# kekeliu-whu/MSF_LOAM

Hardware: AMD Instinct MI355X
Metric: scan-to-map registrations/s (higher is better)
Workload: dtype f64 (f32 kNN distances)

## Files before the change

msf_loam_amd/csrc/msfl_api_slam.inc:

```

#include "msfl_slam.cuh"

namespace {

struct SlamScanBuf {
  DevBuf in_pts, in_ring;
  DevBuf full, fring, curv, label, idx;
  DevBuf cnt;
  DevBuf ex_off;
  DevBuf sharp, ls, ls_ring, flat, lf, lf_ring;
  DevBuf map_ls, map_lf;
  DevBuf full_scan, full_map;
  DevBuf imu;
  int imu_mode = 0;
  DevBuf dqp;
  DevBuf odo_off, odo_status;
  DevBuf poses;
  PinBuf upload;
  int n = 0;
  hipEvent_t ev_odo = nullptr;
  hipEvent_t ev_pose = nullptr, ev_cready = nullptr, ev_match = nullptr, ev_cdone = nullptr;
  DevBuf vox_c, vox_s, vsum_c, vsum_s;
  DevBuf vmeta;
  hipEvent_t ev_feat = nullptr, ev_vox = nullptr;
// ... 119 lines not shown
  r->status_imu = cnt[SC_IMU_BAD] ? MSFL_BAD_ARG : 0;
  cnt[SC_IMU_BAD] = 0;
  r->status_clouds = cnt[SC_CLOUD_BAD] ? MSFL_BAD_ARG : 0;
  cnt[SC_CLOUD_BAD] = 0;
  r->reserved_ = 0;
  r->status_insert = (r->grid_corner[3] | r->grid_corner[4] | r->grid_surf[3] | r->grid_surf[4]) ? MSFL_CAPACITY : 0;
  if (r->odometry.status == 0 && *odo_status != 0) r->odometry.status = *odo_status;
}

msfl_status scan2scan_dyn(msfl_handle* h, const SlamScanBuf& last, const SlamScanBuf& cur, const SlamCaps& caps, double* d_pose, const RegSinks& sinks) {
  hipStream_t st = h->stream;
  const int B = 1;
  const int* d_off = cur.odo_off.as<int>();
  int* d_status = cur.odo_status.as<int>();
  const int n_rec_cap = caps.sharp + caps.flat;
  HIPCHK(h, h->records.reserve(((size_t)4 * caps.flat + (size_t)6 * caps.sharp + 8) * sizeof(double)));
  const BatchView bv = batch_view(cur.sharp.as<float4>(), cur.flat.as<float4>(), d_off + 4, 2, B, n_rec_cap, 0, 0, caps.flat, 1);
  OdomView ov;
  ov.last_ls = last.ls.as<float4>(); ov.last_ls_ring = last.ls_ring.as<uint16_t>(); ov.last_ls_off = d_off;
  ov.last_lf = last.lf.as<float4>(); ov.last_lf_ring = last.lf_ring.as<uint16_t>(); ov.last_lf_off = d_off + 2;
  ov.dist_sq_threshold = h->prm.odom_distance_sq_threshold;
  ov.nearby_scan = h->prm.odom_nearby_scan;
  const SolverParams sp = solver_params(h->prm, h->prm.odom_min_correspondences);
  const bool gate_fits_grid = h->prm.odom_distance_sq_threshold <= 35.9;
  const bool use_grid = gate_fits_grid && !h->odom_force_brute;
  OdomIndex oix{nullptr, nullptr, nullptr, nullptr, std::max(1, div_up(caps.flat, kOdomBlock / kSlamOdomLanes))};
  OdomIndex oie{nullptr, nullptr, nullptr, nullptr, std::max(1, div_up(caps.sharp, kOdomBlock / kSlamOdomLanes))};
  if (use_grid) {
    ScopedTimer timer(h, T_ODOM);
    HIPCHK(h, h->od[OD_TAB].reserve((size_t)B * kOdomTabStride * sizeof(unsigned)));
    HIPCHK(h, h->od[OD_SORTED].reserve((size_t)caps.less_flat * sizeof(float4)));
// ... 18 lines not shown
    ScopedTimer timer(h, T_ODOM);
    hipLaunchKernelGGL(assoc_scan2scan_kernel, dim3(div_up(n_rec_cap, 256), B), dim3(256), 0, st, bv, ov, (const double*)d_pose,
                       (const int*)d_status, h->records.as<double>(), oix.mode, oie.mode);
    if (use_grid) {
      const int plane_blocks = div_up(B, 8) * 8 * oix.tiles, edge_blocks = div_up(B, 8) * 8 * oie.tiles;
      hipLaunchKernelGGL((assoc_scan2scan_grid_kernel<kSlamOdomLanes>), dim3(plane_blocks + edge_blocks), dim3(kOdomBlock), 0, st, bv, ov, oix, oie,
                         plane_blocks, (const double*)d_pose, (const int*)d_status, h->records.as<double>());
    }
    return MSFL_OK;
  });
}

msfl_status scan2map_dyn(msfl_handle* h, const float4* d_corner, const float4* d_surf, const int* d_in_off, int cap_corner, int cap_surf,
                         double* d_pose, int* d_status, const RegSinks& sinks, const DeskewView* deskew = nullptr) {
  const int n_rec_cap = cap_corner + cap_surf;
  HIPCHK(h, h->records.reserve(((size_t)4 * cap_surf + (size_t)6 * cap_corner + 8) * sizeof(double)));
  HIPCHK(h, h->nn.reserve(std::max<size_t>(1, (size_t)n_rec_cap) * 5 * sizeof(int)));
  const BatchView bv = batch_view(d_corner, d_surf, d_in_off, 2, 1, n_rec_cap, 0, 0, cap_surf, 1);
  DeskewView dv{};
  if (deskew) {
    dv = *deskew;
    HIPCHK(h, h->pprime.reserve(std::max<size_t>(1, (size_t)n_rec_cap) * 3 * sizeof(double)));
    dv.pprime = h->pprime.as<double>();
  }
  return solve_outer<kSlamLmBlock>(h, 1, bv, dv.pprime, d_pose, d_status, sinks, solver_params(h->prm, 0), h->prm.outer_iterations, [&](int) {
    s_launch_assoc(h, bv, d_pose, d_status, deskew != nullptr, dv, n_rec_cap);
    return MSFL_OK;
  });
}

constexpr size_t kVoxScratchBytes = (size_t)65536 * 8 + (size_t)2 * 65536 * 2;
// ... 634 lines not shown
```

msf_loam_amd/csrc/msfl_kernels.cuh:

```cuda
#pragma once
#include <hip/hip_runtime.h>
#include <stdint.h>

#include "msfl_math.cuh"

namespace msfl {

#ifndef MSFL_GRID_XSUB
#define MSFL_GRID_XSUB 3
#endif
constexpr int kGridXSub = MSFL_GRID_XSUB;

struct GridDesc {
  float ox, oy, oz;
  float inv_cell;
  float inv_cell_x;
  int dx, dy, dz;
  int n_pts;
  int n_cells;
  int reach;
  int want_cells;
  float cell2, cellx2;
};

// ... 539 lines not shown
  return b;
}
__device__ __forceinline__ int find_scan(const int* __restrict__ rec_off, int n_scans, int g) {
  int lo = 0, hi = n_scans;
  while (hi - lo > 1) {
    const int mid = (lo + hi) >> 1;
    if (rec_off[mid] <= g) lo = mid; else hi = mid;
  }
  return lo;
}

__device__ __forceinline__ size_t feature_slot(const BatchView& bv, bool edge, int f) {
  return edge ? (size_t)(f - bv.c0) : (size_t)(bv.n_records - bv.n_surf_total) + (size_t)(f - bv.s0);
}

__device__ __forceinline__ size_t plane_rec_off(const BatchView& bv, int fi_surf) { return 4 * (size_t)(fi_surf - bv.s0); }
__device__ __forceinline__ size_t edge_rec_off(const BatchView& bv, int fi_corner) {
  return 4 * (size_t)bv.n_surf_total + 6 * (size_t)(fi_corner - bv.c0);
}

struct DeskewView {
  const double* corner_dq; const double* corner_dp;
  const double* surf_dq;   const double* surf_dp;
  const double* V;
  double G[3];
  const double* G_dev;
  double* pprime;
};

#ifndef MSFL_ASSOC_BLOCK
#define MSFL_ASSOC_BLOCK 64
#endif
constexpr int kAssocBlock = MSFL_ASSOC_BLOCK;
// ... 256 lines not shown
    if (DESKEW && fo.ok) {
      static_assert(!DESKEW || KIND == 0, "the de-skew branch runs the per-record kernel");
      const int fd = is_edge ? bv.corner_off[b] + local : bv.surf_off[b] + (local - nc);
      const double dt = (double)(is_edge ? bv.corner[fd].w : bv.surf[fd].w);
      const double* Vb = dv.V + 3 * (size_t)b;
      const double Gv[3] = {dv.G_dev ? dv.G_dev[0] : dv.G[0], dv.G_dev ? dv.G_dev[1] : dv.G[1], dv.G_dev ? dv.G_dev[2] : dv.G[2]};
      fo.C = fo.C - mk3(Vb[0] * dt - 0.5 * Gv[0] * dt * dt, Vb[1] * dt - 0.5 * Gv[1] * dt * dt,
                        Vb[2] * dt - 0.5 * Gv[2] * dt * dt);
    }
  }
  if (is_edge) {
    double* out = rec + edge_rec_off(bv, KIND == 0 ? bv.corner_off[b] + local : fi);
    out[0] = fo.C.x; out[1] = fo.C.y; out[2] = fo.C.z;
    out[3] = fo.N.x; out[4] = fo.N.y; out[5] = fo.N.z;
  } else {
    double* out = rec + plane_rec_off(bv, KIND == 0 ? bv.surf_off[b] + (local - nc) : fi);
    out[0] = fo.N.x; out[1] = fo.N.y; out[2] = fo.N.z; out[3] = dot(fo.N, fo.C);
  }
  if (KIND == 0 && full) {
    double* o = full + 6 * (size_t)g;
    o[0] = fo.C.x; o[1] = fo.C.y; o[2] = fo.C.z; o[3] = fo.N.x; o[4] = fo.N.y; o[5] = fo.N.z;
  }
}

template <bool DESKEW>
__global__ void __launch_bounds__(kAssocBlock, MSFL_FIT_WAVES)
fit_scan2map_kernel(BatchView bv, const float4* __restrict__ map_c, const float4* __restrict__ map_s,
                    const int* __restrict__ nn, double line_ratio, double plane_tol, DeskewView dv,
                    double* __restrict__ rec, double* __restrict__ full) {
  fit_one<DESKEW, 0>(bv, map_c, map_s, nn, line_ratio, plane_tol, dv, rec, full, (int)blockIdx.x);
}
#ifndef MSFL_FIT_SPLIT_WAVES
// ... 7 lines not shown
  else fit_one<false, 2>(bv, map_c, map_s, nn, line_ratio, plane_tol, dv, rec, full, (int)blockIdx.x - edge_blocks);
}

__global__ void __launch_bounds__(256) pack_records_kernel(BatchView bv, const double* __restrict__ full, double* __restrict__ rec) {
  const int g = blockIdx.x * blockDim.x + threadIdx.x;
  if (g >= batch_records(bv)) return;
  const int b = find_scan_wave(bv.rec_off, bv.n_scans, g);
  const int local = g - bv.rec_off[b];
  const int nc = bv.corner_off[b + 1] - bv.corner_off[b];
  const double* in = full + 6 * (size_t)g;
  if (local < nc) {
    double* out = rec + edge_rec_off(bv, bv.corner_off[b] + local);
#pragma unroll
    for (int k = 0; k < 6; k++) out[k] = in[k];
  } else {
    double* out = rec + plane_rec_off(bv, bv.surf_off[b] + (local - nc));
    out[0] = in[3]; out[1] = in[4]; out[2] = in[5]; out[3] = in[3] * in[0] + in[4] * in[1] + in[5] * in[2];
  }
}


struct SolverParams {
  int    max_iterations;
  double huber;
  double radius0, radius_max, radius_min;
  double min_relative_decrease, min_diag, max_diag;
  double ftol, gtol, ptol;
  int    max_invalid;
  int    min_correspondences;
};

struct DevMatchInfo {
// ... 32 lines not shown
#ifndef MSFL_LM_BLOCK
#define MSFL_LM_BLOCK 128
#endif
constexpr int kLmBlock = MSFL_LM_BLOCK;
#ifndef MSFL_ODOM_LM_BLOCK
#define MSFL_ODOM_LM_BLOCK 128
#endif
constexpr int kOdomLmBlock = MSFL_ODOM_LM_BLOCK;
#ifndef MSFL_LM_GROUP_SMALL
#define MSFL_LM_GROUP_SMALL 8
#endif
#ifndef MSFL_LM_GROUP_LARGE
#define MSFL_LM_GROUP_LARGE 4
#endif
constexpr int lm_load_group(int block) { return block >= 512 ? MSFL_LM_GROUP_LARGE : MSFL_LM_GROUP_SMALL; }
constexpr int lm_plane_cache(int block) {
#ifdef MSFL_LM_PLANE_CACHE
  return block == 256 ? MSFL_LM_PLANE_CACHE : block == 128 ? 832 : block == 512 ? 3072 : 384;
#else
  return block == 256 ? 1728 : block == 128 ? 832 : block == 512 ? 3072 : 384;
#endif
}
template <int BLOCK>
struct PlaneCache {
  static constexpr int kPlanes = lm_plane_cache(BLOCK);
  double nx[kPlanes], ny[kPlanes], nz[kPlanes], d0[kPlanes];
  float px[kPlanes], py[kPlanes], pz[kPlanes];
};

constexpr int kEdgeListMax = 1024;
struct EdgeList {
  unsigned mask[kEdgeListMax / 32];
  unsigned short idx[kEdgeListMax];
  int n;
};

#ifdef MSFL_LM_PROFILE
__device__ unsigned long long g_lm_prof[8];
#define LM_T(x) const unsigned long long x = wall_clock64()
#ifndef MSFL_LM_PROFILE_BLOCK
#define MSFL_LM_PROFILE_BLOCK 0
#endif
#define LM_ADD(k, v) if (threadIdx.x == 0 && (MSFL_LM_PROFILE_BLOCK == 0 || MSFL_LM_PROFILE_BLOCK == (int)blockDim.x)) atomicAdd(&g_lm_prof[k], (unsigned long long)(v))
#else
#define LM_T(x)
#define LM_ADD(k, v)
#endif

__device__ __forceinline__ d3 lm_rotate(const quat& q, d3 v) { return quat_rotate(q, v); }

template <int BLOCK, bool FILL>
__device__ __forceinline__ void evaluate_pass(const pose7& T, double huber,
                                              const float4* __restrict__ corner, int nc,
                                              const float4* __restrict__ surf, int ns,
                                              const double* __restrict__ pprime,
                                              const double* __restrict__ rec,
                                              const double* __restrict__ recp,
                                              PlaneCache<BLOCK>& pc, EdgeList& el,
                                              double (&acc)[kAcc], int& n_edge, int& n_plane) {
#pragma unroll
  for (int k = 0; k < kAcc; k++) acc[k] = 0.0;
  n_edge = 0; n_plane = 0;
  const mat3 R = quat_to_matrix(T.q);
  LM_T(t_eval_begin);
  const int n_listed = FILL ? 0 : el.n;
  const int n_walk = FILL ? nc : n_listed + max(nc - kEdgeListMax, 0);
  auto edge_row = [&](int i, d3 C, d3 N, d3 p) __attribute__((always_inline)) {
    if (N.x == 0.0 && N.y == 0.0 && N.z == 0.0) return;
    if (FILL && i < kEdgeListMax) atomicOr(&el.mask[i >> 5], 1u << (i & 31));
    n_edge++;
    const d3 d = mk3(__builtin_fma(R.m[0], p.x, __builtin_fma(R.m[1], p.y, R.m[2] * p.z)) + (T.t.x - C.x),
                     __builtin_fma(R.m[3], p.x, __builtin_fma(R.m[4], p.y, R.m[5] * p.z)) + (T.t.y - C.y),
// ... 7 lines not shown
      w = fmax(2.2250738585072014e-308, huber * inv);
    }
    acc[0] += 0.5 * rho0;
    const d3 l0 = mk3(__builtin_fma(N.y, R.m[6], -(N.z * R.m[3])), __builtin_fma(N.y, R.m[7], -(N.z * R.m[4])), __builtin_fma(N.y, R.m[8], -(N.z * R.m[5])));
    const d3 l1 = mk3(__builtin_fma(N.z, R.m[0], -(N.x * R.m[6])), __builtin_fma(N.z, R.m[1], -(N.x * R.m[7])), __builtin_fma(N.z, R.m[2], -(N.x * R.m[8])));
    const d3 l2 = mk3(__builtin_fma(N.x, R.m[3], -(N.y * R.m[0])), __builtin_fma(N.x, R.m[4], -(N.y * R.m[1])), __builtin_fma(N.x, R.m[5], -(N.y * R.m[2])));
    const d3 b0 = cross(p, l0), b1 = cross(p, l1), b2 = cross(p, l2);
    const double j0[6] = {0.0, -N.z, N.y, b0.x, b0.y, b0.z};
    const double j1[6] = {N.z, 0.0, -N.x, b1.x, b1.y, b1.z};
    const double j2[6] = {-N.y, N.x, 0.0, b2.x, b2.y, b2.z};
    acc_row_w(acc, j0, r.x, w);
    acc_row_w(acc, j1, r.y, w);
    acc_row_w(acc, j2, r.z, w);
  };
  const bool use_cache = (pprime == nullptr);
  auto plane_row = [&](d3 N, double d0, d3 p) __attribute__((always_inline)) {
    if (N.x == 0.0 && N.y == 0.0 && N.z == 0.0) return;
    n_plane++;
    const d3 l = mk3(__builtin_fma(R.m[0], N.x, __builtin_fma(R.m[3], N.y, R.m[6] * N.z)),
                     __builtin_fma(R.m[1], N.x, __builtin_fma(R.m[4], N.y, R.m[7] * N.z)),
                     __builtin_fma(R.m[2], N.x, __builtin_fma(R.m[5], N.y, R.m[8] * N.z)));
    const double nt = __builtin_fma(N.x, T.t.x, __builtin_fma(N.y, T.t.y, __builtin_fma(N.z, T.t.z, -d0)));
    const double r = __builtin_fma(l.x, p.x, __builtin_fma(l.y, p.y, __builtin_fma(l.z, p.z, nt)));
    const d3 b = cross(p, l);
    double rho0, w; huber_weight(huber, r * r, fabs(r), rho0, w);
    acc[0] += 0.5 * rho0;
    const double j[6] = {N.x, N.y, N.z, b.x, b.y, b.z};
    acc_row_w(acc, j, r, w);
  };
  int i = threadIdx.x;
  auto cached_planes = [&]() __attribute__((always_inline)) {
    if (!FILL && use_cache) {
      for (; i < min(ns, PlaneCache<BLOCK>::kPlanes); i += BLOCK)
        plane_row(mk3(pc.nx[i], pc.ny[i], pc.nz[i]), pc.d0[i], mk3((double)pc.px[i], (double)pc.py[i], (double)pc.pz[i]));
    }
  };
  if (pprime == nullptr) {
    constexpr int kEdgeGroup = BLOCK >= 512 ? 1 : 4;
    bool first = true;
    for (int k0 = threadIdx.x; first || k0 < n_walk; k0 += kEdgeGroup * BLOCK) {
      double e6[kEdgeGroup][6];
      float4 ef[kEdgeGroup];
      int ei[kEdgeGroup];
#pragma unroll
      for (int u = 0; u < kEdgeGroup; u++) {
        const int k = min(k0 + u * BLOCK, max(n_walk - 1, 0));
        ei[u] = FILL ? k : (k < n_listed ? (int)el.idx[k] : kEdgeListMax + (k - n_listed));
      }
      if (n_walk > 0) {
// ... 14 lines not shown
  } else {
    for (int k = threadIdx.x; k < n_walk; k += BLOCK) {
      const bool listed = !FILL && k < n_listed;
      const int i = FILL ? k : (listed ? (int)el.idx[k] : kEdgeListMax + (k - n_listed));
      const double* r6 = rec + 6 * (size_t)i;
      const d3 C = mk3(r6[0], r6[1], r6[2]);
      const d3 N = mk3(r6[3], r6[4], r6[5]);
      const d3 p = mk3(pprime[3 * (size_t)i], pprime[3 * (size_t)i + 1], pprime[3 * (size_t)i + 2]);
      edge_row(i, C, N, p);
    }
  }
  LM_T(t_edges_done);
  constexpr int kGroup = lm_load_group(BLOCK);
  if (kGroup > 1 && use_cache) {
    for (; i < ns; i += kGroup * BLOCK) {
      double gn[kGroup][4];
      float4 gf[kGroup];
#pragma unroll
      for (int u = 0; u < kGroup; u++) {
        const int iu = min(i + u * BLOCK, ns - 1);
        const double* r4 = recp + 4 * (size_t)iu;
        gn[u][0] = r4[0]; gn[u][1] = r4[1]; gn[u][2] = r4[2]; gn[u][3] = r4[3];
        gf[u] = surf[iu];
      }
#pragma unroll
      for (int u = 0; u < kGroup; u++) {
        const int iu = i + u * BLOCK;
        if (iu >= ns) break;
        if (FILL && iu < PlaneCache<BLOCK>::kPlanes) {
          pc.nx[iu] = gn[u][0]; pc.ny[iu] = gn[u][1]; pc.nz[iu] = gn[u][2]; pc.d0[iu] = gn[u][3];
          pc.px[iu] = gf[u].x; pc.py[iu] = gf[u].y; pc.pz[iu] = gf[u].z;
        }
        plane_row(mk3(gn[u][0], gn[u][1], gn[u][2]), gn[u][3], mk3((double)gf[u].x, (double)gf[u].y, (double)gf[u].z));
      }
    }
  }
  for (; i < ns; i += BLOCK) {
    const double* r4 = recp + 4 * (size_t)i;
    const d3 N = mk3(r4[0], r4[1], r4[2]); const double d0 = r4[3];
    d3 p;
    if (pprime) { const size_t q = (size_t)(nc + i); p = mk3(pprime[3 * q], pprime[3 * q + 1], pprime[3 * q + 2]); }
    else {
      const float4 f = surf[i];
      p = mk3((double)f.x, (double)f.y, (double)f.z);
      if (FILL && i < PlaneCache<BLOCK>::kPlanes) {
        pc.nx[i] = N.x; pc.ny[i] = N.y; pc.nz[i] = N.z; pc.d0[i] = d0;
        pc.px[i] = f.x; pc.py[i] = f.y; pc.pz[i] = f.z;
      }
    }
    plane_row(N, d0, p);
  }
  LM_T(t_planes_done);
}

struct TrState {
  double sys[kAcc];
  double scale[6], diagonal[6];
  double x[7], cand[7];
  double cost, gmax, x_norm, radius, decrease_factor, model_cost_change;
  int iteration, invalid, successful, reuse_diagonal, step_ok;
};

template <int BLOCK>
struct LmShared {
  double part[BLOCK / 64][kAcc + 2];
// ... 336 lines not shown
```

msf_loam_amd/csrc/msfl_lm_solve_body.inc:

```
  __shared__ LmShared<BLOCK> sh;
  __shared__ PlaneCache<BLOCK> s_cache;
  __shared__ EdgeList s_edges;
#if MSFL_LM_PRIOR
  __shared__ PosePrior s_prior;
#endif
  const int b = blockIdx.x;
  if (status[b] != 0) return;
  if (threadIdx.x < kEdgeListMax / 32) s_edges.mask[threadIdx.x] = 0;
#if MSFL_LM_PRIOR
  int use_prior;
  {
    int bad;
    prior_stage<BLOCK>(prior_all + b, s_prior, bad, use_prior);
    if (bad) {
      if (threadIdx.x == 0) { status[b] = 3; if (info) info[b].status = 3; }
      return;
    }
  }
#endif
  __syncthreads();
  const int nc = bv.corner_off[b + 1] - bv.corner_off[b];
  const int ns = bv.surf_off[b + 1] - bv.surf_off[b];
  const float4* corner = bv.corner + bv.corner_off[b];
  const float4* surf = bv.surf + bv.surf_off[b];
  const size_t r0 = (size_t)bv.rec_off[b];
  const double* rec = rec_all + edge_rec_off(bv, bv.corner_off[b]);
  const double* recp = rec_all + plane_rec_off(bv, bv.surf_off[b]);
  const double* pprime = pprime_all ? pprime_all + 3 * r0 : nullptr;
  double* pose_g = poses + 7 * (size_t)b;
  TrState& tr = sh.tr;
  LM_T(t_begin);
  {
    double acc[kAcc];
    int ne, np;
    const pose7 T = load_pose(pose_g);
    LM_T(t0);
    evaluate_pass<BLOCK, true>(T, prm.huber, corner, nc, surf, ns, pprime, rec, recp, s_cache, s_edges, acc, ne, np);
    LM_T(t1);
    block_reduce<BLOCK>(sh, acc, ne, np);
    LM_T(t2);
    LM_ADD(0, t1 - t0); LM_ADD(1, t2 - t1); LM_ADD(4, 1);
  }
// ... 90 lines not shown
```

msf_loam_amd/csrc/msfl_math.cuh:

```cuda
#pragma once
#include <hip/hip_runtime.h>

namespace msfl {

struct d3 { double x, y, z; };

__device__ __forceinline__ d3 mk3(double x, double y, double z) { d3 r; r.x = x; r.y = y; r.z = z; return r; }
__device__ __forceinline__ d3 operator+(d3 a, d3 b) { return mk3(a.x + b.x, a.y + b.y, a.z + b.z); }
__device__ __forceinline__ d3 operator-(d3 a, d3 b) { return mk3(a.x - b.x, a.y - b.y, a.z - b.z); }
__device__ __forceinline__ d3 operator*(double s, d3 a) { return mk3(s * a.x, s * a.y, s * a.z); }
__device__ __forceinline__ double dot(d3 a, d3 b) { return a.x * b.x + a.y * b.y + a.z * b.z; }
__device__ __forceinline__ d3 cross(d3 a, d3 b) {
  return mk3(a.y * b.z - a.z * b.y, a.z * b.x - a.x * b.z, a.x * b.y - a.y * b.x);
}
__device__ __forceinline__ d3 normalized_rsq(d3 v);
__device__ __forceinline__ d3 normalized(d3 v) {
  const double z = dot(v, v);
  if (z > 0.0) { const double s = sqrt(z); return mk3(v.x / s, v.y / s, v.z / s); }
  return v;
}

#ifndef MSFL_IEEE_DIV
#define MSFL_IEEE_DIV 0
#endif
// ... 7 lines not shown
}
__device__ __forceinline__ double fast_rsqrt(double x) {
  if (MSFL_IEEE_DIV || !(x > 1e-280 && x < 1e280)) return 1.0 / sqrt(x);
  double y = __builtin_amdgcn_rsq(x);
  const double hx = 0.5 * x;
  double e = __builtin_fma(-hx * y, y, 0.5);
  y = __builtin_fma(y, e, y);
  e = __builtin_fma(-hx * y, y, 0.5);
  return __builtin_fma(y, e, y);
}

__device__ __forceinline__ d3 normalized_rsq(d3 v) {
  const double z = dot(v, v);
  if (!MSFL_IEEE_DIV && z > 1e-280 && z < 1e280) { const double s = fast_rsqrt(z); return mk3(v.x * s, v.y * s, v.z * s); }
  return normalized(v);
}

struct quat { double x, y, z, w; };
struct pose7 { d3 t; quat q; };

__device__ __forceinline__ pose7 load_pose(const double* __restrict__ p) {
  pose7 r;
  r.t = mk3(p[0], p[1], p[2]);
  r.q.x = p[3]; r.q.y = p[4]; r.q.z = p[5]; r.q.w = p[6];
  return r;
}
__device__ __forceinline__ void store_pose(double* __restrict__ p, const pose7& a) {
  p[0] = a.t.x; p[1] = a.t.y; p[2] = a.t.z; p[3] = a.q.x; p[4] = a.q.y; p[5] = a.q.z; p[6] = a.q.w;
}

// ... 235 lines not shown
```

msf_loam_amd/csrc/msfl_odom.cuh:

```cuda
#pragma once
#include <hip/hip_runtime.h>
#include <stdint.h>

#include "msfl_kernels.cuh"

namespace msfl {

__device__ __forceinline__ d3 odom_unit(d3 v) { return normalized_rsq(v); }
__device__ __forceinline__ d3 odom_centroid3(d3 a, d3 b, d3 c) {
  const double third = 1.0 / 3.0;
  return mk3((a.x + b.x + c.x) * third, (a.y + b.y + c.y) * third, (a.z + b.z + c.z) * third);
}

struct OdomView {
  const float4* last_ls; const uint16_t* last_ls_ring; const int* last_ls_off;
  const float4* last_lf; const uint16_t* last_lf_ring; const int* last_lf_off;
  double dist_sq_threshold;
  double nearby_scan;
};

constexpr int kOdomTile = 1024;

__device__ __forceinline__ float odom_dist(float4 a, float3 q) {
  const msfl_f2 axy = {a.x, a.y}, qxy = {q.x, q.y};
// ... 3 lines not shown
  return sxy.x + sxy.y + dz * dz;
}

__global__ void __launch_bounds__(256)
assoc_scan2scan_kernel(BatchView bv, OdomView ov, const double* __restrict__ poses, const int* __restrict__ status,
                       double* __restrict__ rec, const int* __restrict__ plane_mode, const int* __restrict__ edge_mode) {
  __shared__ float4 s_tile[kOdomTile];
  const int b = blockIdx.y;
  const int n_sharp = bv.corner_off[b + 1] - bv.corner_off[b];
  const int n_flat = bv.surf_off[b + 1] - bv.surf_off[b];
  const int nq = n_sharp + n_flat;
  const int q0 = blockIdx.x * 256;
  if (q0 >= nq) return;
  const int qi = q0 + threadIdx.x;
  const bool has_q = qi < nq;
  double* out = rec + (qi < n_sharp ? edge_rec_off(bv, bv.corner_off[b] + qi) : plane_rec_off(bv, bv.surf_off[b] + (qi - n_sharp)));
  const int out_len = qi < n_sharp ? 6 : 4;
  if (status[b] != 0) {
    if (has_q) for (int k = 0; k < out_len; k++) out[k] = 0.0;
    return;
  }
  const bool planes_here = plane_mode == nullptr || plane_mode[b] != 0;
  const bool edges_here = edge_mode == nullptr || edge_mode[b] != 0;
  const bool is_edge = has_q && qi < n_sharp && edges_here;
  const bool is_plane = has_q && qi >= n_sharp && planes_here;
  float4 f = make_float4(0, 0, 0, 0);
  float3 q = make_float3(0, 0, 0);
  if (is_edge || is_plane) {
    f = is_edge ? bv.corner[bv.corner_off[b] + qi] : bv.surf[bv.surf_off[b] + (qi - n_sharp)];
    const pose7 T = load_pose(poses + 7 * b);
    q = transform_point_f32(T, f.x, f.y, f.z);
  }
  const float thr = (float)ov.dist_sq_threshold;
  const bool wg_has_edge = q0 < n_sharp && edges_here;
// ... 82 lines not shown
          const float4 a = tp[closest], c = tp[min2];
          const d3 A = mk3((double)a.x, (double)a.y, (double)a.z), Bp = mk3((double)c.x, (double)c.y, (double)c.z);
          N = odom_unit(A - Bp);
          C = A;
        }
      } else {
        if (min2 >= 0 && min3 >= 0) {
          const float4 a = tp[closest], c = tp[min2], e = tp[min3];
          const d3 A = mk3((double)a.x, (double)a.y, (double)a.z), Bp = mk3((double)c.x, (double)c.y, (double)c.z),
                   Cp = mk3((double)e.x, (double)e.y, (double)e.z);
          N = odom_unit(cross(A - Bp, A - Cp));
          C = odom_centroid3(A, Bp, Cp);
        }
      }
      if (edge_pass) { out[0] = C.x; out[1] = C.y; out[2] = C.z; out[3] = N.x; out[4] = N.y; out[5] = N.z; }
      else { out[0] = N.x; out[1] = N.y; out[2] = N.z; out[3] = dot(N, C); }
    } else if (mine) {
      for (int k = 0; k < out_len; k++) out[k] = 0.0;
    }
  }
}

struct DJ { float d; int j; };
__device__ __forceinline__ DJ wave_min_lo(DJ v) {
#pragma unroll
  for (int o = 32; o > 0; o >>= 1) {
    const float d = __shfl_xor(v.d, o); const int j = __shfl_xor(v.j, o);
    if (d < v.d || (d == v.d && j < v.j)) { v.d = d; v.j = j; }
  }
  return v;
}
__device__ __forceinline__ DJ wave_min_hi(DJ v) {
#pragma unroll
// ... 2 lines not shown
    if (j >= 0 && (v.j < 0 || d < v.d || (d == v.d && j > v.j))) { v.d = d; v.j = j; }
  }
  return v;
}

__global__ void __launch_bounds__(256)
assoc_scan2scan_wave_kernel(BatchView bv, OdomView ov, const double* __restrict__ poses, const int* __restrict__ status,
                            double* __restrict__ rec) {
  const int b = blockIdx.y;
  const int lane = threadIdx.x & 63;
  const int n_sharp = bv.corner_off[b + 1] - bv.corner_off[b];
  const int n_flat = bv.surf_off[b + 1] - bv.surf_off[b];
  const int qi = blockIdx.x * 4 + (threadIdx.x >> 6);
  if (qi >= n_sharp + n_flat) return;
  const bool edge = qi < n_sharp;
  double* out = rec + (edge ? edge_rec_off(bv, bv.corner_off[b] + qi) : plane_rec_off(bv, bv.surf_off[b] + (qi - n_sharp)));
  const int out_len = edge ? 6 : 4;
  const float4* tp = edge ? ov.last_ls + ov.last_ls_off[b] : ov.last_lf + ov.last_lf_off[b];
  const uint16_t* tr = edge ? ov.last_ls_ring + ov.last_ls_off[b] : ov.last_lf_ring + ov.last_lf_off[b];
  const int nt = edge ? ov.last_ls_off[b + 1] - ov.last_ls_off[b] : ov.last_lf_off[b + 1] - ov.last_lf_off[b];
  const float thr = (float)ov.dist_sq_threshold;
  bool ok = status[b] == 0 && nt > 0;
  float3 q = make_float3(0, 0, 0);
  int closest = -1;
  if (ok) {
    const float4 f = edge ? bv.corner[bv.corner_off[b] + qi] : bv.surf[bv.surf_off[b] + (qi - n_sharp)];
    q = transform_point_f32(load_pose(poses + 7 * b), f.x, f.y, f.z);
    DJ best{INFINITY, 0x7fffffff};
    for (int j = lane; j < nt; j += 64) {
      const float d = odom_dist(tp[j], q);
      if (d < best.d) { best.d = d; best.j = j; }
    }
    best = wave_min_lo(best);
    ok = best.j != 0x7fffffff && best.d < thr;
    closest = best.j;
  }
  if (!ok) {
    if (lane < out_len) out[lane] = 0.0;
    return;
  }
  const int id = tr[closest];
  const float hi_ring = (float)id + (float)ov.nearby_scan, lo_ring = (float)id - (float)ov.nearby_scan;
  int fwd_end = nt, back_end = -1;
  for (int j = lane; j < nt; j += 64) {
    const float rj = (float)tr[j];
    if (j > closest && rj > hi_ring) fwd_end = min(fwd_end, j);
    if (j < closest && rj < lo_ring) back_end = max(back_end, j);
  }
#pragma unroll
  for (int o = 32; o > 0; o >>= 1) { fwd_end = min(fwd_end, __shfl_xor(fwd_end, o)); back_end = max(back_end, __shfl_xor(back_end, o)); }
  DJ f2{thr, 0x7fffffff}, f3{thr, 0x7fffffff}, b2{thr, -1}, b3{thr, -1};
  for (int j = lane; j < nt; j += 64) {
    if (j == closest || j >= fwd_end || j <= back_end) continue;
// ... 23 lines not shown
  if (edge) {
    if (min2 >= 0) {
      const float4 a = tp[closest], c = tp[min2];
      const d3 A = mk3((double)a.x, (double)a.y, (double)a.z), Bp = mk3((double)c.x, (double)c.y, (double)c.z);
      N = odom_unit(A - Bp); C = A;
    }
    out[0] = C.x; out[1] = C.y; out[2] = C.z; out[3] = N.x; out[4] = N.y; out[5] = N.z;
  } else {
    if (min2 >= 0 && min3 >= 0) {
      const float4 a = tp[closest], c = tp[min2], e = tp[min3];
      const d3 A = mk3((double)a.x, (double)a.y, (double)a.z), Bp = mk3((double)c.x, (double)c.y, (double)c.z),
               Cp = mk3((double)e.x, (double)e.y, (double)e.z);
      N = odom_unit(cross(A - Bp, A - Cp));
      C = odom_centroid3(A, Bp, Cp);
    }
    out[0] = N.x; out[1] = N.y; out[2] = N.z; out[3] = dot(N, C);
  }
}

constexpr int kOdomRange = 512;
constexpr int kOdomMaxCells = 40960;
constexpr int kOdomTabStride = kOdomMaxCells + 1;
#ifndef MSFL_ODOM_LANES
#define MSFL_ODOM_LANES 16
#endif
constexpr int kOdomLanes = MSFL_ODOM_LANES;
#ifndef MSFL_ODOM_BLOCK
#define MSFL_ODOM_BLOCK 64
#endif
constexpr int kOdomBlock = MSFL_ODOM_BLOCK;
constexpr int kOdomLevels = 5;
// ... 365 lines not shown

template <int L, bool EDGE>
__device__ __forceinline__ void odom_grid_query(const BatchView& bv, const OdomView& ov, const OdomIndex& ix, const double* __restrict__ poses,
                                                const int* __restrict__ status, double* __restrict__ rec, int block) {
  const int tiles = ix.tiles;
  const int group = block / (8 * tiles), within = block - group * (8 * tiles);
  const int b = group * 8 + (within & 7);
  const int tile = within >> 3;
  if (b >= bv.n_scans) return;
  if (ix.mode[b] != 0) return;
  const int n_sharp = bv.corner_off[b + 1] - bv.corner_off[b];
  const int n_flat = bv.surf_off[b + 1] - bv.surf_off[b];
  const int sl = threadIdx.x % L;
  const int qf = tile * (kOdomBlock / L) + threadIdx.x / L;
  if (qf >= (EDGE ? n_sharp : n_flat)) return;
  constexpr int kOut = EDGE ? 6 : 4;
  double* out = rec + (EDGE ? edge_rec_off(bv, bv.corner_off[b] + qf) : plane_rec_off(bv, bv.surf_off[b] + qf));
  const int* t_off = EDGE ? ov.last_ls_off : ov.last_lf_off;
  const int s0 = t_off[b], s1 = t_off[b + 1];
  const float4* tp = (EDGE ? ov.last_ls : ov.last_lf) + s0;
  const float thr = (float)ov.dist_sq_threshold;
  bool ok = status[b] == 0 && s1 > s0;
  float3 q = make_float3(0, 0, 0);
  if (ok) {
    const float4 f = EDGE ? bv.corner[bv.corner_off[b] + qf] : bv.surf[bv.surf_off[b] + qf];
    q = transform_point_f32(load_pose(poses + 7 * b), f.x, f.y, f.z);
    ok = fabsf(q.x) < (float)(kOdomRange + 7) && fabsf(q.y) < (float)(kOdomRange + 7);
  }
  if (!ok) { if (sl < kOut) out[sl] = 0.0; return; }
  const float fx = floorf(q.x), fy = floorf(q.y);
  const OdomPairDesc pd = ix.desc[b];
  const int cx = (int)fx - pd.ox, cy = (int)fy - pd.oy;
  const unsigned* tab = ix.tab + (size_t)b * kOdomTabStride;
  const float4* sorted = ix.sorted + s0;
  int b0[3], b1[3];
  odom_runs3(tab, pd.W, pd.H, cx, cy, b0, b1);
  unsigned long long kbest = ~0ull;
  auto nearest = [&](const float4 p) __attribute__((always_inline)) {
    const unsigned long long k = ((unsigned long long)__float_as_uint(odom_dist(p, q)) << 32) | (unsigned)__float_as_int(p.w);
    kbest = k < kbest ? k : kbest;
  };
  int l1 = 0;
  for (int l = 0; l < kOdomLevels; l++) {
    const int r = odom_level_radius(l);
    l1 = l;
    if (l == 0) odom_walk_runs3<L>(sorted, b0, b1, sl, nearest);
    else odom_walk<L>(tab, sorted, pd.W, pd.H, cx, cy, r, sl, nearest);
    kbest = group_min_key<L>(kbest);
    if (__uint_as_float((unsigned)(kbest >> 32)) < odom_gap_sq(q, fx, fy, r)) break;
  }
  if (!(__uint_as_float((unsigned)(kbest >> 32)) < thr)) { if (sl < kOut) out[sl] = 0.0; return; }
  const int closest = (int)((unsigned)kbest & 0xffffffu), id = (int)((unsigned)kbest >> 24 & 0xffu);
  const float hi_ring = (float)id + (float)ov.nearby_scan, lo_ring = (float)id - (float)ov.nearby_scan;
  const int hi_i = hi_ring == hi_ring ? (int)fminf(fmaxf(floorf(hi_ring), -1048576.f), 1048576.f) : 1048576;
  const int lo_i = lo_ring == lo_ring ? (int)fminf(fmaxf(ceilf(lo_ring), -1048576.f), 1048576.f) : -1048576;
  const bool window = hi_i >= lo_i;
  const unsigned span = window ? (unsigned)(hi_i - lo_i) : 0u;
  const int lo_w = window ? lo_i : (1 << 22);
  const unsigned long long none = (unsigned long long)__float_as_uint(thr) << 32;
  unsigned long long k2, k3;
  auto windowed = [&](const float4 p) __attribute__((always_inline)) {
    const int w = __float_as_int(p.w), j = w & 0xffffff, rj = (int)((unsigned)w >> 24);
    const int t = j - closest;
    const bool same = rj == id;
    const bool skip = (unsigned)(rj - lo_w) > span || t == 0 || (EDGE && same);
    const float d = odom_dist(p, q);
// ... 29 lines not shown
      const float4 a = tp[closest], c = tp[min2];
      const d3 A = mk3((double)a.x, (double)a.y, (double)a.z), Bp = mk3((double)c.x, (double)c.y, (double)c.z);
      N = odom_unit(A - Bp);
      C = A;
    }
    out[0] = C.x; out[1] = C.y; out[2] = C.z; out[3] = N.x; out[4] = N.y; out[5] = N.z;
    return;
  }
  if (min2 >= 0 && min3 >= 0) {
    const float4 a = tp[closest], c = tp[min2], e = tp[min3];
    const d3 A = mk3((double)a.x, (double)a.y, (double)a.z), Bp = mk3((double)c.x, (double)c.y, (double)c.z),
             Cp = mk3((double)e.x, (double)e.y, (double)e.z);
    N = odom_unit(cross(A - Bp, A - Cp));
    C = odom_centroid3(A, Bp, Cp);
  }
  out[0] = N.x; out[1] = N.y; out[2] = N.z; out[3] = dot(N, C);
}

template <int L>
__global__ void __launch_bounds__(kOdomBlock)
assoc_scan2scan_grid_kernel(BatchView bv, OdomView ov, OdomIndex ix_plane, OdomIndex ix_edge, int plane_blocks,
                            const double* __restrict__ poses, const int* __restrict__ status, double* __restrict__ rec) {
  if ((int)blockIdx.x < plane_blocks) odom_grid_query<L, false>(bv, ov, ix_plane, poses, status, rec, (int)blockIdx.x);
  else odom_grid_query<L, true>(bv, ov, ix_edge, poses, status, rec, (int)blockIdx.x - plane_blocks);
}

}
```

msf_loam_amd/csrc/msfl_uncertainty_body.inc:

```
  static_assert(BLOCK >= 64, "36 lanes assemble the matrices");
  __shared__ LmShared<BLOCK> sh;
  __shared__ PlaneCache<BLOCK> s_cache;
  __shared__ EdgeList s_edges;
  __shared__ UncRecord s_out;
  const int b = blockIdx.x;
#if MSFL_UNC_PRIOR
  __shared__ PosePrior s_prior;
  int use_prior;
  {
    int bad;
    prior_stage<BLOCK>(prior_all + b, s_prior, bad, use_prior);
  }
#endif
  unsigned long long* s_words = reinterpret_cast<unsigned long long*>(&s_out);
  for (int i = threadIdx.x; i < kUncWords; i += BLOCK) s_words[i] = 0ull;
  if (threadIdx.x < kEdgeListMax / 32) s_edges.mask[threadIdx.x] = 0;
  __syncthreads();
  bool valid = false;
  if (status[b] == 0) {
    const int nc = bv.corner_off[b + 1] - bv.corner_off[b];
    const int ns = bv.surf_off[b + 1] - bv.surf_off[b];
    const float4* corner = bv.corner + bv.corner_off[b];
    const float4* surf = bv.surf + bv.surf_off[b];
    const double* rec = rec_all + edge_rec_off(bv, bv.corner_off[b]);
    const double* recp = rec_all + plane_rec_off(bv, bv.surf_off[b]);
    const double* pprime = pprime_all ? pprime_all + 3 * (size_t)bv.rec_off[b] : nullptr;
    double acc[kAcc];
    int ne, np;
    const pose7 T = load_pose(poses + 7 * (size_t)b);
    evaluate_pass<BLOCK, true>(T, huber, corner, nc, surf, ns, pprime, rec, recp, s_cache, s_edges, acc, ne, np);
    block_reduce<BLOCK>(sh, acc, ne, np);
#if MSFL_UNC_PRIOR
    if (use_prior && threadIdx.x == 0) prior_accumulate(T, &s_prior, sh.red);
#endif
    __syncthreads();
    const int n_edge = sh.cnt[0], n_plane = sh.cnt[1];
    valid = (n_edge + n_plane >= min_correspondences) && (n_edge + n_plane > 0);
    if (valid) {
      if (threadIdx.x < 36) {
        const int i = threadIdx.x / 6, j = threadIdx.x % 6;
// ... 49 lines not shown
```

Baseline: 934,900.

## Compress plane records to two-component normal plus offset and cache only points

Plane correspondence records shrink from four doubles (normal plus offset) to three: two normal components with the dropped-axis code packed into exponent bits, stored as a double2 array plus a separate offset array, with the third component rebuilt by a sqrt on read. The LM shared-memory plane cache now holds only float point coordinates by default, so more planes fit and the normal is read from global memory instead. The aim is less record traffic in the LM and uncertainty passes. In exchange, each plane row pays decode and sqrt work, the normal loses some precision through reconstruction, and reads of normals from global memory may cost more than the old shared-memory reads.

Result: slower. 899,000 (-3.8%).

```diff
diff --git a/msf_loam_amd/csrc/msfl_api_slam.inc b/msf_loam_amd/csrc/msfl_api_slam.inc
--- a/msf_loam_amd/csrc/msfl_api_slam.inc
+++ b/msf_loam_amd/csrc/msfl_api_slam.inc
@@ -157,7 +157,7 @@
   const int* d_off = cur.odo_off.as<int>();
   int* d_status = cur.odo_status.as<int>();
   const int n_rec_cap = caps.sharp + caps.flat;
-  HIPCHK(h, h->records.reserve(((size_t)4 * caps.flat + (size_t)6 * caps.sharp + 8) * sizeof(double)));
+  HIPCHK(h, h->records.reserve(((size_t)3 * caps.flat + (size_t)6 * caps.sharp + 8) * sizeof(double)));
   const BatchView bv = batch_view(cur.sharp.as<float4>(), cur.flat.as<float4>(), d_off + 4, 2, B, n_rec_cap, 0, 0, caps.flat, 1);
   OdomView ov;
   ov.last_ls = last.ls.as<float4>(); ov.last_ls_ring = last.ls_ring.as<uint16_t>(); ov.last_ls_off = d_off;
@@ -206,7 +206,7 @@
 msfl_status scan2map_dyn(msfl_handle* h, const float4* d_corner, const float4* d_surf, const int* d_in_off, int cap_corner, int cap_surf,
                          double* d_pose, int* d_status, const RegSinks& sinks, const DeskewView* deskew = nullptr) {
   const int n_rec_cap = cap_corner + cap_surf;
-  HIPCHK(h, h->records.reserve(((size_t)4 * cap_surf + (size_t)6 * cap_corner + 8) * sizeof(double)));
+  HIPCHK(h, h->records.reserve(((size_t)3 * cap_surf + (size_t)6 * cap_corner + 8) * sizeof(double)));
   HIPCHK(h, h->nn.reserve(std::max<size_t>(1, (size_t)n_rec_cap) * 5 * sizeof(int)));
   const BatchView bv = batch_view(d_corner, d_surf, d_in_off, 2, 1, n_rec_cap, 0, 0, cap_surf, 1);
   DeskewView dv{};
diff --git a/msf_loam_amd/csrc/msfl_kernels.cuh b/msf_loam_amd/csrc/msfl_kernels.cuh
--- a/msf_loam_amd/csrc/msfl_kernels.cuh
+++ b/msf_loam_amd/csrc/msfl_kernels.cuh
@@ -577,9 +577,29 @@
   return edge ? (size_t)(f - bv.c0) : (size_t)(bv.n_records - bv.n_surf_total) + (size_t)(f - bv.s0);
 }
 
-__device__ __forceinline__ size_t plane_rec_off(const BatchView& bv, int fi_surf) { return 4 * (size_t)(fi_surf - bv.s0); }
+struct PlaneRecPtr { double2* ab; double* d0; };
+struct PlaneRecCPtr { const double2* ab; const double* d0; };
+__device__ __forceinline__ PlaneRecPtr plane_rec_ptr(const BatchView& bv, double* rec, int fi_surf) {
+  PlaneRecPtr p;
+  p.ab = reinterpret_cast<double2*>(rec) + (size_t)(fi_surf - bv.s0);
+  p.d0 = rec + 2 * (size_t)bv.n_surf_total + (size_t)(fi_surf - bv.s0);
+  return p;
+}
+__device__ __forceinline__ PlaneRecCPtr plane_rec_ptr(const BatchView& bv, const double* rec, int fi_surf) {
+  PlaneRecCPtr p;
+  p.ab = reinterpret_cast<const double2*>(rec) + (size_t)(fi_surf - bv.s0);
+  p.d0 = rec + 2 * (size_t)bv.n_surf_total + (size_t)(fi_surf - bv.s0);
+  return p;
+}
 __device__ __forceinline__ size_t edge_rec_off(const BatchView& bv, int fi_corner) {
-  return 4 * (size_t)bv.n_surf_total + 6 * (size_t)(fi_corner - bv.c0);
+  return 3 * (size_t)bv.n_surf_total + 6 * (size_t)(fi_corner - bv.c0);
+}
+__device__ __forceinline__ d3 store_plane_record(const PlaneRecPtr& out, d3 N, d3 C) {
+  PlaneRec r; d3 Nu; bool neg;
+  plane_encode(N, C, r, Nu, neg);
+  *out.ab = make_double2(r.a, r.b);
+  *out.d0 = r.d0;
+  return neg ? mk3(-Nu.x, -Nu.y, -Nu.z) : Nu;
 }
 
 struct DeskewView {
@@ -866,8 +886,7 @@
     out[0] = fo.C.x; out[1] = fo.C.y; out[2] = fo.C.z;
     out[3] = fo.N.x; out[4] = fo.N.y; out[5] = fo.N.z;
   } else {
-    double* out = rec + plane_rec_off(bv, KIND == 0 ? bv.surf_off[b] + (local - nc) : fi);
-    out[0] = fo.N.x; out[1] = fo.N.y; out[2] = fo.N.z; out[3] = dot(fo.N, fo.C);
+    fo.N = store_plane_record(plane_rec_ptr(bv, rec, KIND == 0 ? bv.surf_off[b] + (local - nc) : fi), fo.N, fo.C);
   }
   if (KIND == 0 && full) {
     double* o = full + 6 * (size_t)g;
@@ -905,8 +924,7 @@
 #pragma unroll
     for (int k = 0; k < 6; k++) out[k] = in[k];
   } else {
-    double* out = rec + plane_rec_off(bv, bv.surf_off[b] + (local - nc));
-    out[0] = in[3]; out[1] = in[4]; out[2] = in[5]; out[3] = in[3] * in[0] + in[4] * in[1] + in[5] * in[2];
+    store_plane_record(plane_rec_ptr(bv, rec, bv.surf_off[b] + (local - nc)), normalized(mk3(in[3], in[4], in[5])), mk3(in[0], in[1], in[2]));
   }
 }
 
@@ -969,19 +987,30 @@
 #define MSFL_LM_GROUP_LARGE 4
 #endif
 constexpr int lm_load_group(int block) { return block >= 512 ? MSFL_LM_GROUP_LARGE : MSFL_LM_GROUP_SMALL; }
+#ifndef MSFL_LM_CACHE_POINTS
+#define MSFL_LM_CACHE_POINTS 1
+#endif
+constexpr bool kLmCachePoints = MSFL_LM_CACHE_POINTS != 0;
+constexpr int lm_cache_bytes(int block) { return block == 256 ? 76032 : block == 128 ? 36608 : block == 512 ? 135168 : 16896; }
 constexpr int lm_plane_cache(int block) {
 #ifdef MSFL_LM_PLANE_CACHE
-  return block == 256 ? MSFL_LM_PLANE_CACHE : block == 128 ? 832 : block == 512 ? 3072 : 384;
-#else
-  return block == 256 ? 1728 : block == 128 ? 832 : block == 512 ? 3072 : 384;
+  if (block == 256) return MSFL_LM_PLANE_CACHE;
 #endif
-}
+  return lm_cache_bytes(block) / (kLmCachePoints ? 12 : 36);
+}
+template <int BLOCK, bool POINTS> struct PlaneCacheT;
 template <int BLOCK>
-struct PlaneCache {
+struct PlaneCacheT<BLOCK, true> {
   static constexpr int kPlanes = lm_plane_cache(BLOCK);
-  double nx[kPlanes], ny[kPlanes], nz[kPlanes], d0[kPlanes];
   float px[kPlanes], py[kPlanes], pz[kPlanes];
 };
+template <int BLOCK>
+struct PlaneCacheT<BLOCK, false> {
+  static constexpr int kPlanes = lm_plane_cache(BLOCK);
+  double a[kPlanes], b[kPlanes], d0[kPlanes];
+  float px[kPlanes], py[kPlanes], pz[kPlanes];
+};
+template <int BLOCK> using PlaneCache = PlaneCacheT<BLOCK, kLmCachePoints>;
 
 constexpr int kEdgeListMax = 1024;
 struct EdgeList {
@@ -1010,7 +1039,7 @@
                                               const float4* __restrict__ surf, int ns,
                                               const double* __restrict__ pprime,
                                               const double* __restrict__ rec,
-                                              const double* __restrict__ recp,
+                                              PlaneRecCPtr recp,
                                               PlaneCache<BLOCK>& pc, EdgeList& el,
                                               double (&acc)[kAcc], int& n_edge, int& n_plane) {
 #pragma unroll
@@ -1048,8 +1077,11 @@
     acc_row_w(acc, j2, r.z, w);
   };
   const bool use_cache = (pprime == nullptr);
-  auto plane_row = [&](d3 N, double d0, d3 p) __attribute__((always_inline)) {
-    if (N.x == 0.0 && N.y == 0.0 && N.z == 0.0) return;
+  const double2* __restrict__ rab = recp.ab;
+  const double* __restrict__ rd0 = recp.d0;
+  auto plane_row = [&](double ra, double rb, double d0, d3 p) __attribute__((always_inline)) {
+    d3 N;
+    if (!plane_decode(ra, rb, N)) return;
     n_plane++;
     const d3 l = mk3(__builtin_fma(R.m[0], N.x, __builtin_fma(R.m[3], N.y, R.m[6] * N.z)),
                      __builtin_fma(R.m[1], N.x, __builtin_fma(R.m[4], N.y, R.m[7] * N.z)),
@@ -1064,9 +1096,11 @@
   };
   int i = threadIdx.x;
   auto cached_planes = [&]() __attribute__((always_inline)) {
-    if (!FILL && use_cache) {
-      for (; i < min(ns, PlaneCache<BLOCK>::kPlanes); i += BLOCK)
-        plane_row(mk3(pc.nx[i], pc.ny[i], pc.nz[i]), pc.d0[i], mk3((double)pc.px[i], (double)pc.py[i], (double)pc.pz[i]));
+    if constexpr (!kLmCachePoints) {
+      if (!FILL && use_cache) {
+        for (; i < min(ns, PlaneCache<BLOCK>::kPlanes); i += BLOCK)
+          plane_row(pc.a[i], pc.b[i], pc.d0[i], mk3((double)pc.px[i], (double)pc.py[i], (double)pc.pz[i]));
+      }
     }
   };
   if (pprime == nullptr) {
@@ -1111,41 +1145,48 @@
   constexpr int kGroup = lm_load_group(BLOCK);
   if (kGroup > 1 && use_cache) {
     for (; i < ns; i += kGroup * BLOCK) {
-      double gn[kGroup][4];
-      float4 gf[kGroup];
+      double gn[kGroup][3];
+      float gp[kGroup][3];
 #pragma unroll
       for (int u = 0; u < kGroup; u++) {
         const int iu = min(i + u * BLOCK, ns - 1);
-        const double* r4 = recp + 4 * (size_t)iu;
-        gn[u][0] = r4[0]; gn[u][1] = r4[1]; gn[u][2] = r4[2]; gn[u][3] = r4[3];
-        gf[u] = surf[iu];
+        const double2 ab = rab[iu];
+        gn[u][0] = ab.x; gn[u][1] = ab.y; gn[u][2] = rd0[iu];
+        if (kLmCachePoints && !FILL && iu < PlaneCache<BLOCK>::kPlanes) {
+          gp[u][0] = pc.px[iu]; gp[u][1] = pc.py[iu]; gp[u][2] = pc.pz[iu];
+        } else {
+          const float4 f = surf[iu];
+          gp[u][0] = f.x; gp[u][1] = f.y; gp[u][2] = f.z;
+        }
       }
 #pragma unroll
       for (int u = 0; u < kGroup; u++) {
         const int iu = i + u * BLOCK;
         if (iu >= ns) break;
         if (FILL && iu < PlaneCache<BLOCK>::kPlanes) {
-          pc.nx[iu] = gn[u][0]; pc.ny[iu] = gn[u][1]; pc.nz[iu] = gn[u][2]; pc.d0[iu] = gn[u][3];
-          pc.px[iu] = gf[u].x; pc.py[iu] = gf[u].y; pc.pz[iu] = gf[u].z;
+          if constexpr (!kLmCachePoints) { pc.a[iu] = gn[u][0]; pc.b[iu] = gn[u][1]; pc.d0[iu] = gn[u][2]; }
+          pc.px[iu] = gp[u][0]; pc.py[iu] = gp[u][1]; pc.pz[iu] = gp[u][2];
         }
-        plane_row(mk3(gn[u][0], gn[u][1], gn[u][2]), gn[u][3], mk3((double)gf[u].x, (double)gf[u].y, (double)gf[u].z));
+        plane_row(gn[u][0], gn[u][1], gn[u][2], mk3((double)gp[u][0], (double)gp[u][1], (double)gp[u][2]));
       }
     }
   }
   for (; i < ns; i += BLOCK) {
-    const double* r4 = recp + 4 * (size_t)i;
-    const d3 N = mk3(r4[0], r4[1], r4[2]); const double d0 = r4[3];
+    const double2 ab = rab[i];
+    const double d0 = rd0[i];
     d3 p;
     if (pprime) { const size_t q = (size_t)(nc + i); p = mk3(pprime[3 * q], pprime[3 * q + 1], pprime[3 * q + 2]); }
     else {
-      const float4 f = surf[i];
-      p = mk3((double)f.x, (double)f.y, (double)f.z);
+      float px, py, pz;
+      if (kLmCachePoints && !FILL && i < PlaneCache<BLOCK>::kPlanes) { px = pc.px[i]; py = pc.py[i]; pz = pc.pz[i]; }
+      else { const float4 f = surf[i]; px = f.x; py = f.y; pz = f.z; }
+      p = mk3((double)px, (double)py, (double)pz);
       if (FILL && i < PlaneCache<BLOCK>::kPlanes) {
-        pc.nx[i] = N.x; pc.ny[i] = N.y; pc.nz[i] = N.z; pc.d0[i] = d0;
-        pc.px[i] = f.x; pc.py[i] = f.y; pc.pz[i] = f.z;
+        if constexpr (!kLmCachePoints) { pc.a[i] = ab.x; pc.b[i] = ab.y; pc.d0[i] = d0; }
+        pc.px[i] = px; pc.py[i] = py; pc.pz[i] = pz;
       }
     }
-    plane_row(N, d0, p);
+    plane_row(ab.x, ab.y, d0, p);
   }
   LM_T(t_planes_done);
 }
diff --git a/msf_loam_amd/csrc/msfl_lm_solve_body.inc b/msf_loam_amd/csrc/msfl_lm_solve_body.inc
--- a/msf_loam_amd/csrc/msfl_lm_solve_body.inc
+++ b/msf_loam_amd/csrc/msfl_lm_solve_body.inc
@@ -25,7 +25,7 @@
   const float4* surf = bv.surf + bv.surf_off[b];
   const size_t r0 = (size_t)bv.rec_off[b];
   const double* rec = rec_all + edge_rec_off(bv, bv.corner_off[b]);
-  const double* recp = rec_all + plane_rec_off(bv, bv.surf_off[b]);
+  const PlaneRecCPtr recp = plane_rec_ptr(bv, rec_all, bv.surf_off[b]);
   const double* pprime = pprime_all ? pprime_all + 3 * r0 : nullptr;
   double* pose_g = poses + 7 * (size_t)b;
   TrState& tr = sh.tr;
diff --git a/msf_loam_amd/csrc/msfl_math.cuh b/msf_loam_amd/csrc/msfl_math.cuh
--- a/msf_loam_amd/csrc/msfl_math.cuh
+++ b/msf_loam_amd/csrc/msfl_math.cuh
@@ -45,6 +45,44 @@
   const double z = dot(v, v);
   if (!MSFL_IEEE_DIV && z > 1e-280 && z < 1e280) { const double s = fast_rsqrt(z); return mk3(v.x * s, v.y * s, v.z * s); }
   return normalized(v);
+}
+
+struct PlaneRec { double a, b, d0; };
+
+__device__ __forceinline__ double plane_dropped(double a, double b) {
+  const double aa = a * a, bb = b * b;
+  return sqrt((1.0 - aa) - bb);
+}
+
+constexpr int kPlaneFlagBit = 1 << 30;
+
+__device__ __forceinline__ bool plane_encode(d3 N, d3 C, PlaneRec& out, d3& N_used, bool& negated) {
+  out.a = 0.0; out.b = 0.0; out.d0 = 0.0; N_used = mk3(0, 0, 0); negated = false;
+  if (N.x == 0.0 && N.y == 0.0 && N.z == 0.0) return false;
+  const double ax = fabs(N.x), ay = fabs(N.y), az = fabs(N.z);
+  const int k = (ax >= ay && ax >= az) ? 0 : (ay >= az ? 1 : 2);
+  const double nk = k == 0 ? N.x : k == 1 ? N.y : N.z;
+  negated = nk < 0.0;
+  if (negated) N = mk3(-N.x, -N.y, -N.z);
+  const double a = k == 0 ? N.y : k == 1 ? N.z : N.x;
+  const double b = k == 0 ? N.z : k == 1 ? N.x : N.y;
+  const double c = plane_dropped(a, b);
+  N_used = k == 0 ? mk3(c, a, b) : k == 1 ? mk3(b, c, a) : mk3(a, b, c);
+  const int code = k + 1;
+  out.a = __hiloint2double(__double2hiint(a) | ((code & 1) ? kPlaneFlagBit : 0), __double2loint(a));
+  out.b = __hiloint2double(__double2hiint(b) | ((code & 2) ? kPlaneFlagBit : 0), __double2loint(b));
+  out.d0 = dot(N_used, C);
+  return true;
+}
+
+__device__ __forceinline__ bool plane_decode(double ra, double rb, d3& N) {
+  const int ha = __double2hiint(ra), hb = __double2hiint(rb);
+  const int code = ((ha >> 30) & 1) | (((hb >> 30) & 1) << 1);
+  const double a = __hiloint2double(ha & ~kPlaneFlagBit, __double2loint(ra));
+  const double b = __hiloint2double(hb & ~kPlaneFlagBit, __double2loint(rb));
+  const double c = plane_dropped(a, b);
+  N = code == 1 ? mk3(c, a, b) : code == 2 ? mk3(b, c, a) : mk3(a, b, c);
+  return code != 0;
 }
 
 struct quat { double x, y, z, w; };
diff --git a/msf_loam_amd/csrc/msfl_odom.cuh b/msf_loam_amd/csrc/msfl_odom.cuh
--- a/msf_loam_amd/csrc/msfl_odom.cuh
+++ b/msf_loam_amd/csrc/msfl_odom.cuh
@@ -41,10 +41,14 @@
   if (q0 >= nq) return;
   const int qi = q0 + threadIdx.x;
   const bool has_q = qi < nq;
-  double* out = rec + (qi < n_sharp ? edge_rec_off(bv, bv.corner_off[b] + qi) : plane_rec_off(bv, bv.surf_off[b] + (qi - n_sharp)));
-  const int out_len = qi < n_sharp ? 6 : 4;
+  double* out = rec + edge_rec_off(bv, bv.corner_off[b] + qi);
+  auto outp = [&]() { return plane_rec_ptr(bv, rec, bv.surf_off[b] + (qi - n_sharp)); };
+  auto reject = [&]() {
+    if (qi < n_sharp) { for (int k = 0; k < 6; k++) out[k] = 0.0; }
+    else store_plane_record(outp(), mk3(0, 0, 0), mk3(0, 0, 0));
+  };
   if (status[b] != 0) {
-    if (has_q) for (int k = 0; k < out_len; k++) out[k] = 0.0;
+    if (has_q) reject();
     return;
   }
   const bool planes_here = plane_mode == nullptr || plane_mode[b] != 0;
@@ -157,9 +161,9 @@
         }
       }
       if (edge_pass) { out[0] = C.x; out[1] = C.y; out[2] = C.z; out[3] = N.x; out[4] = N.y; out[5] = N.z; }
-      else { out[0] = N.x; out[1] = N.y; out[2] = N.z; out[3] = dot(N, C); }
+      else store_plane_record(outp(), N, C);
     } else if (mine) {
-      for (int k = 0; k < out_len; k++) out[k] = 0.0;
+      reject();
     }
   }
 }
@@ -192,8 +196,8 @@
   const int qi = blockIdx.x * 4 + (threadIdx.x >> 6);
   if (qi >= n_sharp + n_flat) return;
   const bool edge = qi < n_sharp;
-  double* out = rec + (edge ? edge_rec_off(bv, bv.corner_off[b] + qi) : plane_rec_off(bv, bv.surf_off[b] + (qi - n_sharp)));
-  const int out_len = edge ? 6 : 4;
+  double* out = rec + edge_rec_off(bv, bv.corner_off[b] + qi);
+  auto outp = [&]() { return plane_rec_ptr(bv, rec, bv.surf_off[b] + (qi - n_sharp)); };
   const float4* tp = edge ? ov.last_ls + ov.last_ls_off[b] : ov.last_lf + ov.last_lf_off[b];
   const uint16_t* tr = edge ? ov.last_ls_ring + ov.last_ls_off[b] : ov.last_lf_ring + ov.last_lf_off[b];
   const int nt = edge ? ov.last_ls_off[b + 1] - ov.last_ls_off[b] : ov.last_lf_off[b + 1] - ov.last_lf_off[b];
@@ -214,7 +218,8 @@
     closest = best.j;
   }
   if (!ok) {
-    if (lane < out_len) out[lane] = 0.0;
+    if (edge) { if (lane < 6) out[lane] = 0.0; }
+    else if (lane == 0) store_plane_record(outp(), mk3(0, 0, 0), mk3(0, 0, 0));
     return;
   }
   const int id = tr[closest];
@@ -268,7 +273,7 @@
       N = odom_unit(cross(A - Bp, A - Cp));
       C = odom_centroid3(A, Bp, Cp);
     }
-    out[0] = N.x; out[1] = N.y; out[2] = N.z; out[3] = dot(N, C);
+    store_plane_record(outp(), N, C);
   }
 }
 
@@ -664,8 +669,12 @@
   const int sl = threadIdx.x % L;
   const int qf = tile * (kOdomBlock / L) + threadIdx.x / L;
   if (qf >= (EDGE ? n_sharp : n_flat)) return;
-  constexpr int kOut = EDGE ? 6 : 4;
-  double* out = rec + (EDGE ? edge_rec_off(bv, bv.corner_off[b] + qf) : plane_rec_off(bv, bv.surf_off[b] + qf));
+  double* out = rec + edge_rec_off(bv, bv.corner_off[b] + qf);
+  auto outp = [&]() { return plane_rec_ptr(bv, rec, bv.surf_off[b] + qf); };
+  auto reject = [&]() {
+    if (EDGE) { if (sl < 6) out[sl] = 0.0; }
+    else if (sl == 0) store_plane_record(outp(), mk3(0, 0, 0), mk3(0, 0, 0));
+  };
   const int* t_off = EDGE ? ov.last_ls_off : ov.last_lf_off;
   const int s0 = t_off[b], s1 = t_off[b + 1];
   const float4* tp = (EDGE ? ov.last_ls : ov.last_lf) + s0;
@@ -677,7 +686,7 @@
     q = transform_point_f32(load_pose(poses + 7 * b), f.x, f.y, f.z);
     ok = fabsf(q.x) < (float)(kOdomRange + 7) && fabsf(q.y) < (float)(kOdomRange + 7);
   }
-  if (!ok) { if (sl < kOut) out[sl] = 0.0; return; }
+  if (!ok) { reject(); return; }
   const float fx = floorf(q.x), fy = floorf(q.y);
   const OdomPairDesc pd = ix.desc[b];
   const int cx = (int)fx - pd.ox, cy = (int)fy - pd.oy;
@@ -699,7 +708,7 @@
     kbest = group_min_key<L>(kbest);
     if (__uint_as_float((unsigned)(kbest >> 32)) < odom_gap_sq(q, fx, fy, r)) break;
   }
-  if (!(__uint_as_float((unsigned)(kbest >> 32)) < thr)) { if (sl < kOut) out[sl] = 0.0; return; }
+  if (!(__uint_as_float((unsigned)(kbest >> 32)) < thr)) { reject(); return; }
   const int closest = (int)((unsigned)kbest & 0xffffffu), id = (int)((unsigned)kbest >> 24 & 0xffu);
   const float hi_ring = (float)id + (float)ov.nearby_scan, lo_ring = (float)id - (float)ov.nearby_scan;
   const int hi_i = hi_ring == hi_ring ? (int)fminf(fmaxf(floorf(hi_ring), -1048576.f), 1048576.f) : 1048576;
@@ -759,7 +768,7 @@
     N = odom_unit(cross(A - Bp, A - Cp));
     C = odom_centroid3(A, Bp, Cp);
   }
-  out[0] = N.x; out[1] = N.y; out[2] = N.z; out[3] = dot(N, C);
+  store_plane_record(outp(), N, C);
 }
 
 template <int L>
diff --git a/msf_loam_amd/csrc/msfl_uncertainty_body.inc b/msf_loam_amd/csrc/msfl_uncertainty_body.inc
--- a/msf_loam_amd/csrc/msfl_uncertainty_body.inc
+++ b/msf_loam_amd/csrc/msfl_uncertainty_body.inc
@@ -23,7 +23,7 @@
     const float4* corner = bv.corner + bv.corner_off[b];
     const float4* surf = bv.surf + bv.surf_off[b];
     const double* rec = rec_all + edge_rec_off(bv, bv.corner_off[b]);
-    const double* recp = rec_all + plane_rec_off(bv, bv.surf_off[b]);
+    const PlaneRecCPtr recp = plane_rec_ptr(bv, rec_all, bv.surf_off[b]);
     const double* pprime = pprime_all ? pprime_all + 3 * (size_t)bv.rec_off[b] : nullptr;
     double acc[kAcc];
     int ne, np;
```
